# ndoll1998/lightgrad

Hardware: AMD Instinct MI355X
Metric: mnist_mlp_train_steps_per_sec_batch1024_per_gpu (higher is better)
Workload: dtype f32; 1 GPU; mnist_mlp_784x512x10_bias_batch1024_mse_adabelief_lr1e-3 (fwd+bwd+allreduce+optimizer); batch_per_gpu=1024, global_batch=1024, parallelism=dp1, optimizer_kernel=fused, input_requires_grad=True, dispatch=hipGraph replay (python tape captured once; 13 consecutive steps per graph), steps_per_graph=13, device=AMD Instinct (gfx950), compute_units=256, clock_mhz=2400

## Files before the change

include/lghip.h:

```cpp
#ifndef LGHIP_H
#define LGHIP_H

#include <stddef.h>
#include <stdint.h>

#ifdef __cplusplus
extern "C" {
#endif

#define LG_MAX_DIMS 8

#define LG_OK            0
#define LG_EINVAL       -1
#define LG_EHIP         -2
#define LG_ENOMEM       -3
#define LG_ENOTINIT     -4
#define LG_ECOMM        -5
#define LG_EINDEX       -6

const char* lg_last_error(void);

int lg_device_count(int* count);
int lg_init(int device);
int lg_device(int* device);
// ... 221 lines not shown
                              const float* mask, int64_t sbm);
int lg_attention_long_bwd_f32(const float* q, int64_t ldq, int64_t sbq, const float* k, int64_t ldk, int64_t sbk,
                              const float* v, int64_t ldv, int64_t sbv, const float* g, int64_t ldg, int64_t sbg,
                              const float* p, float* dq, int64_t lddq, int64_t sbdq, float* dk, int64_t lddk, int64_t sbdk,
                              float* dv, int64_t lddv, int64_t sbdv, int64_t batch, int64_t heads, int64_t S, int64_t D,
                              float scale);

int lg_attention_dropout_supported(int64_t S, int64_t D);
int lg_attention_dropout_fwd_f32(const float* q, int64_t ldq, int64_t sbq, const float* k, int64_t ldk, int64_t sbk,
                                 const float* v, int64_t ldv, int64_t sbv, float* o, int64_t ldo, int64_t sbo, float* p,
                                 int64_t batch, int64_t heads, int64_t S, int64_t D, float scale,
                                 const float* mask, int64_t sbm, double prob, uint64_t* base_out);
int lg_attention_dropout_bwd_f32(const float* q, int64_t ldq, int64_t sbq, const float* k, int64_t ldk, int64_t sbk,
                                 const float* v, int64_t ldv, int64_t sbv, const float* g, int64_t ldg, int64_t sbg,
                                 const float* p, float* dq, int64_t lddq, int64_t sbdq, float* dk, int64_t lddk, int64_t sbdk,
                                 float* dv, int64_t lddv, int64_t sbdv, int64_t batch, int64_t heads, int64_t S, int64_t D,
                                 float scale, double prob, const uint64_t* base);

int lg_gemm_pair_begin(void);
int lg_gemm_pair_end(void);
int lg_gemm_pair_mse_loss(const float* row_loss, int64_t rows, int64_t n, float* loss);
int lg_gemm_pair_hold(void);
int lg_gemm_pair_resume(void);

int lg_gemm_group_begin(void);
int lg_gemm_group_colsum_f32(const float* in, int64_t ld, int64_t rows, int64_t cols, float* out, int accumulate);
int lg_gemm_group_flush(void);
int lg_gemm_group_end(void);

int lg_head_fwd_f32(const float* x, int64_t ldx, int relu, const float* w, const float* bias, const float* target,
                    float* y, float* err, float* row_loss, int64_t rows, int64_t hidden, int64_t outs);
int lg_head_fwd_grad_f32(const float* x, int64_t ldx, int relu, const float* w, const float* bias, const float* target,
                         float* y, float* err, float* row_loss, float* dx, float* gpre, int64_t rows, int64_t hidden, int64_t outs);
int lg_gemm_bias_head_fwd_f32(const float* x, int64_t ldx, const float* w1, int64_t ldw1, const float* b1, float* pre,
                              int64_t rows, int64_t hidden, int64_t d_in, int relu,
                              const float* w2, const float* b2, const float* target, float* y, float* err, float* row_loss,
                              float* dx, float* gpre, int64_t outs, int chain, int* launches);
int lg_mse_finalize_f32(const float* row_loss, int64_t rows, int64_t n, float* loss);
int lg_head_bwd_f32(const float* x, int64_t ldx, int relu, const float* g, const float* w,
                    float* dx, float* gpre, float* dw, int dw_accumulate, float* db, int db_accumulate,
                    int64_t rows, int64_t hidden, int64_t outs, const float* row_loss, float* loss);

int lg_softmax_f32(const float* x, float* y, int64_t rows, int64_t cols);
int lg_softmax_bwd_f32(const float* y, const float* g, float* dx, int64_t rows, int64_t cols);
int lg_softmax_scaled_f32(const float* x, float* y, int64_t rows, int64_t cols, float scale);
int lg_softmax_scaled_bwd_f32(const float* y, const float* g, float* dx, int64_t rows, int64_t cols, float scale);
// ... 59 lines not shown
```

lightgrad_amd/autograd/hip/lib.py:

```python
import ctypes
import os
from ctypes import c_int, c_int64, c_uint32, c_uint64, c_size_t, c_float, c_double, c_void_p, c_char_p, POINTER

_PKG_DIR = os.path.dirname(os.path.dirname(os.path.dirname(os.path.abspath(__file__))))
LIB_PATH = os.environ.get("LIGHTGRAD_HIP_LIB") or os.path.join(_PKG_DIR, "liblghip.so")
COMM_LIB_PATH = os.path.join(_PKG_DIR, "liblghip_comm.so")

ACT_GELU, ACT_GELU_BWD = 1, 2
EW_COPY, EW_NEG, EW_EXP, EW_LOG, EW_RELU, EW_SIGMOID, EW_TANH, EW_SIN, EW_COS, EW_SQRT, EW_GELU = range(11)
(EW_ADD, EW_SUB, EW_MUL, EW_DIV, EW_POW, EW_RELU_BWD, EW_SIGMOID_BWD, EW_TANH_BWD, EW_LOG_BWD,
 EW_SIN_BWD, EW_COS_BWD, EW_EQ, EW_GE, EW_BIAS_RELU, EW_GELU_BWD) = range(32, 47)
EW_MAX_BWD, EW_FMA = 64, 65
EW_MUL_BWD, EW_DIV_BWD, EW_POW_BWD = 96, 97, 98
RED_SUM, RED_MAX, RED_MIN = 0, 1, 2
DT_I16, DT_I32, DT_I64, DT_F64, DT_F32 = 1, 2, 3, 4, 5


class DeviceInfo(ctypes.Structure):
    _fields_ = [("name", ctypes.c_char * 128), ("arch", ctypes.c_char * 32),
                ("compute_units", ctypes.c_int32), ("clock_mhz", ctypes.c_int32),
                ("wavefront_size", ctypes.c_int32), ("lds_bytes_per_cu", ctypes.c_int32),
                ("hbm_bytes", ctypes.c_uint64), ("l2_bytes", ctypes.c_int32), ("reserved", ctypes.c_int32)]


# ... 30 lines not shown
    "lg_fill_strided": (c_int, [c_int, c_int, _I64P, c_void_p, _I64P, c_uint64]),
    "lg_ew": (c_int, [c_int, c_int, _I64P, c_void_p, _I64P, c_void_p, _I64P,
                      c_void_p, _I64P, c_void_p, _I64P, c_void_p, _I64P, c_void_p, _I64P, c_float]),
    "lg_ew_last_plan": (c_int, [POINTER(ctypes.c_int32)]),
    "lg_reduce": (c_int, [c_int, c_int, _I64P, c_void_p, _I64P, c_uint32, c_void_p]),
    "lg_ew_typed": (c_int, [c_int, c_int, c_int, _I64P, c_void_p, _I64P, c_void_p, _I64P, c_void_p, _I64P, c_double, c_int64]),
    "lg_reduce_typed": (c_int, [c_int, c_int, c_int, _I64P, c_void_p, _I64P, c_uint32, c_void_p]),
    "lg_cast": (c_int, [c_int, c_int, c_int, _I64P, c_void_p, _I64P, c_void_p, _I64P]),
    "lg_reduce_acc": (c_int, [c_int, c_int, _I64P, c_void_p, _I64P, c_uint32, c_void_p, c_int]),
    "lg_reduce_last_plan": (c_int, [POINTER(ctypes.c_int32)]),
    "lg_argreduce_f32": (c_int, [c_int, c_int, _I64P, c_void_p, _I64P, c_int, c_void_p]),
    "lg_argreduce_last_plan": (c_int, [POINTER(ctypes.c_int32)]),
    "lg_top1_count_f32": (c_int, [c_void_p, c_int64, c_int64, c_void_p, c_int, c_int, c_int64, c_int, c_void_p]),
    "lg_gemm_f32": (c_int, [c_int, c_int, c_int64, c_int64, c_int64, c_void_p, c_int64, c_int64,
                            c_void_p, c_int64, c_int64, c_void_p, c_int64, c_int64, c_int64, c_int]),
    "lg_gemm_bf16_f32": (c_int, [c_int, c_int, c_int64, c_int64, c_int64, c_void_p, c_int64, c_void_p, c_int64, c_void_p, c_int64,
                                 c_void_p, c_int]),
    "lg_bf16_round_f32": (c_int, [c_void_p, c_void_p, c_int64]),
    "lg_gemm_pair_begin": (c_int, []),
    "lg_gemm_pair_end": (c_int, []),
    "lg_gemm_pair_mse_loss": (c_int, [c_void_p, c_int64, c_int64, c_void_p]),
    "lg_gemm_pair_hold": (c_int, []),
    "lg_gemm_pair_resume": (c_int, []),
    "lg_gemm_group_begin": (c_int, []),
    "lg_gemm_group_colsum_f32": (c_int, [c_void_p, c_int64, c_int64, c_int64, c_void_p, c_int]),
    "lg_gemm_group_flush": (c_int, []),
    "lg_gemm_group_end": (c_int, []),
    "lg_adam_step_f32": (c_int, [c_void_p, c_void_p, c_void_p, c_void_p, c_int64, c_double, c_double, c_double,
                                 c_double, c_double, c_double, c_double, c_int]),
    "lg_adam_step_dev_f32": (c_int, [c_void_p, c_void_p, c_void_p, c_void_p, c_int64, c_double, c_double, c_double,
                                     c_double, c_void_p, c_int64, c_int64, c_double, c_int]),
    "lg_counter_add_i64": (c_int, [c_void_p, c_int64]),
    "lg_adam_multi_dev_f32": (c_int, [c_void_p, c_void_p, c_void_p, c_void_p, c_int, _I64P, c_double, c_double, c_double,
                                      c_double, c_void_p, c_int64, c_double, c_int]),
    "lg_grad_norm_clip_f32": (c_int, [c_void_p, c_int64, c_double, c_double, c_void_p, c_void_p, c_void_p]),
    "lg_adamw_multi_dev_f32": (c_int, [c_void_p, c_void_p, c_void_p, c_void_p, c_int, _I64P, c_double, c_double, c_double,
                                       c_double, c_void_p, c_int64, c_double, c_int, c_double, c_char_p, c_void_p, c_int, c_int64, c_int64]),
    "lg_adam_plan_create": (c_int, [POINTER(c_void_p), c_void_p, c_void_p, c_void_p, c_void_p, c_int64, c_void_p, c_void_p, c_int64, c_int64,
                                    c_double, c_double, c_double, c_double, c_double, c_int]),
    "lg_adam_plan_destroy": (c_int, [c_void_p]),
    "lg_adam_epilogue_arm": (c_int, [c_void_p, c_int64, c_void_p]),
    "lg_adam_epilogue_finish": (c_int, [POINTER(c_int), POINTER(c_int)]),
    "lg_adam_epilogue_disarm": (c_int, []),
    "lg_gemm_bias_f32": (c_int, [c_int, c_int, c_int64, c_int64, c_int64, c_void_p, c_int64, c_int64,
                                 c_void_p, c_int64, c_int64, c_void_p, c_int64, c_int64, c_int64, c_void_p]),
    "lg_gemm_addend_f32": (c_int, [c_int, c_int, c_int64, c_int64, c_int64, c_void_p, c_int64, c_void_p, c_int64, c_void_p, c_int64,
# ... 180 lines not shown
```

lightgrad_amd/csrc/gemm.hip:

```cpp
#include "common.h"
#include "gelu_common.h"
#include "adam_common.h"
#include "tail_jobs.h"
#include "mse_finalize.h"
#include "head_fwd_body.h"
#include <cstdlib>
#include <cstring>
#include <type_traits>

namespace lg {

typedef float f32x16 __attribute__((ext_vector_type(16)));
typedef unsigned int u32x4 __attribute__((ext_vector_type(4)));
typedef float f32x4 __attribute__((ext_vector_type(4)));

#ifndef LG_SMALL_PD
#define LG_SMALL_PD 2
#endif
constexpr int kSmallTilePrefetch = LG_SMALL_PD;
#ifndef LG_WAVE_PRIVATE_PD
#define LG_WAVE_PRIVATE_PD 1
#endif
constexpr int kWavePrivatePrefetch = LG_WAVE_PRIVATE_PD;

// ... 3 lines not shown
};
static FastDiv make_fastdiv(int64_t d) {
    if (d < 1) d = 1;
    uint32_t l = 0;
    while ((int64_t(1) << l) < d) ++l;
    FastDiv f;
    f.m = uint32_t((uint64_t(1) << (31 + l)) / uint64_t(d) + 1);
    f.s = 31 + l;
    return f;
}

struct GemmArgs {
    const float* A;
    const float* B;
    float*       C;
    int64_t M, N, K;
    int64_t lda, ldb, ldc;
    int64_t sA, sB, sC;
    int64_t sA2, sB2, sC2;
    int     batch_inner;
    int     tiles_m, tiles_n;
    int     nwg;
    int     accumulate;
    const float* bias;
    const float* addend;
    int64_t      ldadd;
    int     group_m;
    int     k_slices;
    int64_t k_per_slice;
    float*  W;
    int*    tickets;
    float*  rowsum;
    int     rowsum_accumulate;
    FastDiv div_per_batch, div_slices, div_gspan, div_group, div_last_group, div_batch_inner;
    int     k_tail;
    short   relu_a, relu_b;
    int     act;
    float*  aux;
    int     multi;
    int64_t boff[3], coff[3], biasoff[3];
    int     seg_k, seg_steps;
    int64_t seg_jump[2];
    const AdamPlan* adam_c;
    const AdamPlan* adam_r;
#ifdef LG_GEMM_TIMELINE
    unsigned long long* tl;
// ... 84 lines not shown
            while (__hip_atomic_load(flag, __ATOMIC_RELAXED, __HIP_MEMORY_SCOPE_AGENT) == 0) {
                __builtin_amdgcn_s_sleep(2);
                if (wall_clock64() - t0 > 200000000ull) {
                    __hip_atomic_fetch_or(c.status, LG_STATUS_HANDOFF_TIMEOUT, __ATOMIC_RELAXED, __HIP_MEMORY_SCOPE_SYSTEM);
                    ok = 0;
                    break;
                }
            }
            seen = ok;
        }
        __syncthreads();
        __builtin_amdgcn_fence(__ATOMIC_ACQUIRE, "wavefront");
        const int64_t row = row0 + wave;
        if (row < a.rows) head_fwd_row<OMAX, true>(a, lds, row, lane);
        if (tid == 0 && seen) {
            if (__hip_atomic_fetch_add(done, 1, __ATOMIC_RELAXED, __HIP_MEMORY_SCOPE_AGENT) == readers - 1) {
                __hip_atomic_store(done, 0, __ATOMIC_RELAXED, __HIP_MEMORY_SCOPE_AGENT);
                __hip_atomic_store(flag, 0, __ATOMIC_RELAXED, __HIP_MEMORY_SCOPE_AGENT);
            }
        }
    }
}

template <int PD, bool SECOND_BKC = false>
__global__ void __launch_bounds__(256) sgemm_pair_wgrad_xgrad(GemmArgs first, GemmArgs second) {
    constexpr int L1 = gemm_lds_floats<64, 64, 32, false, false, 1>(), L2 = gemm_lds_floats<64, 64, 32, true, SECOND_BKC, 1>();
    __shared__ __attribute__((aligned(16))) float lds[L1 > L2 ? L1 : L2];
    constexpr int BM = 64, BN = 64, BK = 32, WM = 2, WN = 2, KG = 1, XT = 0;
    constexpr bool VA = true, VB = true;
#define LG_TILE_OWNS_LDS 0
    if (int(blockIdx.x) < first.nwg) {
        constexpr bool AKC = false, BKC = false;
        const GemmArgs& g = first;
#define LG_TILE_BID int(blockIdx.x)
#include "gemm_tile_body.inc"
#undef LG_TILE_BID
    } else {
        constexpr bool AKC = true, BKC = SECOND_BKC;
        const GemmArgs& g = second;
#define LG_TILE_BID (int(blockIdx.x) - first.nwg)
#include "gemm_tile_body.inc"
#undef LG_TILE_BID
    }
#undef LG_TILE_OWNS_LDS
}

int lg_mse_finalize_job(const float* row_loss, int64_t rows, float inv_n, float* loss);
struct PairFirsts { GemmArgs w[2]; };
struct LossJob {
    const float* row_loss;
    float*       loss;
    int64_t      rows;
    float        inv_n;
};
template <int PD>
__global__ void __launch_bounds__(256) sgemm_triple_wgrad2_xgrad(PairFirsts firsts, GemmArgs second, LossJob job) {
    constexpr int L1 = gemm_lds_floats<64, 64, 32, false, false, 1>(), L2 = gemm_lds_floats<64, 64, 32, true, false, 1>();
    __shared__ __attribute__((aligned(16))) float lds[L1 > L2 ? L1 : L2];
    constexpr int BM = 64, BN = 64, BK = 32, WM = 2, WN = 2, KG = 1, XT = 0;
    constexpr bool VA = true, VB = true;
#define LG_TILE_OWNS_LDS 0
    const int n0w = firsts.w[0].nwg, n1w = firsts.w[1].nwg;
    if (int(blockIdx.x) < n0w + n1w) {
        constexpr bool AKC = false, BKC = false;
        const int which = int(blockIdx.x) >= n0w ? 1 : 0;
        const GemmArgs g = firsts.w[which];
#define LG_TILE_BID (int(blockIdx.x) - (which ? n0w : 0))
#include "gemm_tile_body.inc"
#undef LG_TILE_BID
    } else if (int(blockIdx.x) < n0w + n1w + second.nwg) {
        constexpr bool AKC = true, BKC = false;
        const GemmArgs& g = second;
#define LG_TILE_BID (int(blockIdx.x) - n0w - n1w)
#include "gemm_tile_body.inc"
#undef LG_TILE_BID
    } else {
        finalize_loss(job.row_loss, job.rows, job.inv_n, job.loss, lds);
    }
#undef LG_TILE_OWNS_LDS
}

constexpr int kGroupMax = 14;
struct GroupProduct {
    const float* A;
    const float* B;
    float*       C;
    float*       W;
    int*         tickets;
    float*       rowsum;
    int64_t      M, N, K, lda, ldb, ldc, k_per_slice;
    int          tiles_m, tiles_n, nwg, accumulate, group_m, k_slices, rowsum_accumulate, k_tail;
    FastDiv      div_per_batch, div_slices, div_gspan, div_group, div_last_group, div_batch_inner;
// ... 43 lines not shown
        int64_t r = q;
        for (; r + 28 < grp.cs_rows; r += 32) {
#pragma unroll
            for (int e = 0; e < 8; ++e) acc[e] += in[(r + 4 * e) * grp.cs_ld];
        }
        for (; r < grp.cs_rows; r += 4) acc[0] += in[r * grp.cs_ld];
        lds[threadIdx.x] = ((acc[0] + acc[1]) + (acc[2] + acc[3])) + ((acc[4] + acc[5]) + (acc[6] + acc[7]));
        __syncthreads();
        if (q == 0 && live) {
            const float v = (lds[cl] + lds[64 + cl]) + (lds[128 + cl] + lds[192 + cl]);
            grp.cs_out[col] = grp.cs_accumulate ? grp.cs_out[col] + v : v;
        }
        return;
    }
    const int bid = int(blockIdx.x) - grp.cs_wgs;
    if (bid >= grp.first[grp.count]) {
        tail_group_body(grp.tail, bid - grp.first[grp.count]);
        return;
    }
    int which = 0;
    while (which + 1 < grp.count && bid >= grp.first[which + 1]) ++which;
    const GemmArgs g = unpack_product(grp.p[which]);
#define LG_TILE_OWNS_LDS 0
#define LG_TILE_BID (bid - grp.first[which])
#include "gemm_tile_body.inc"
#undef LG_TILE_BID
#undef LG_TILE_OWNS_LDS
}

template <int BM, int BN, int BK, int WM, int WN, bool AKC, bool BKC, int KG>
static void launch_layout(const GemmArgs& g, bool va, bool vb) {
    dim3 grid(g.nwg), block(WM * WN * KG * 64);
    hipStream_t s = rt().stream;
    constexpr int PD = (BM * BN <= 64 * 64) ? kSmallTilePrefetch : 2;
    static_assert(BM * BN < 256 * 256 || PD <= 2, "a third K-tile in flight does not fit the 256x256 tile's 128 registers: ring registers would spill while their loads are in flight");
    if constexpr (kWavePrivateTile<BM, BN, WM, WN, KG> && AKC && BKC) {
        static const char* kloop_env = getenv("LG_GEMM_KLOOP");
        if (va && vb && !(kloop_env && strcmp(kloop_env, "coop") == 0)) {
            constexpr int WPD = kWavePrivatePrefetch;
            if (g.multi) hipLaunchKernelGGL((sgemm_mfma<BM, BN, BK, WM, WN, true, true, true, true, WPD, KG, 1, true>), grid, block, 0, s, g);
            else         hipLaunchKernelGGL((sgemm_mfma<BM, BN, BK, WM, WN, true, true, true, true, WPD, KG, 0, true>), grid, block, 0, s, g);
            return;
        }
    }
    if constexpr (kHasExtras<BM, BN>) {
        if constexpr (AKC && BKC)  { if (g.multi) { hipLaunchKernelGGL((sgemm_mfma<BM, BN, BK, WM, WN, AKC, BKC, true, true, PD, KG, 1>), grid, block, 0, s, g); return; } }
        if constexpr (AKC && !BKC) { if (g.seg_k) { hipLaunchKernelGGL((sgemm_mfma<BM, BN, BK, WM, WN, AKC, BKC, true, true, PD, KG, 2>), grid, block, 0, s, g); return; } }
    }
    if constexpr (!kHasExtras<BM, BN>) {
        hipLaunchKernelGGL((sgemm_mfma<BM, BN, BK, WM, WN, AKC, BKC, true, true, PD, KG>), grid, block, 0, s, g);
        return;
    }
    if (va && vb)  hipLaunchKernelGGL((sgemm_mfma<BM, BN, BK, WM, WN, AKC, BKC, true, true, PD, KG>), grid, block, 0, s, g);
    else if (va)   hipLaunchKernelGGL((sgemm_mfma<BM, BN, BK, WM, WN, AKC, BKC, true, false, 1, KG>), grid, block, 0, s, g);
    else if (vb)   hipLaunchKernelGGL((sgemm_mfma<BM, BN, BK, WM, WN, AKC, BKC, false, true, 1, KG>), grid, block, 0, s, g);
    else           hipLaunchKernelGGL((sgemm_mfma<BM, BN, BK, WM, WN, AKC, BKC, false, false, 1, KG>), grid, block, 0, s, g);
}

#ifdef LG_GEMM_TIMELINE
static void lg_debug_timeline_state(unsigned long long* buf, int nwg, int slices, int tiles);
#endif
struct PairState {
    int      active = 0;
    int      count = 0;
    bool     second_bkc = false;
    GemmArgs args[3];
    bool     is_s[3] = {false, false, false};
    int64_t  batch[3] = {1, 1, 1};
    int64_t  tiles = 0;
    LossJob  job{};
};
static PairState& pair_state() { static PairState p; return p; }

static void pair_launch_single(const GemmArgs& g, bool is_s) {
    dim3 grid(g.nwg), block(256);
    constexpr int PD = kSmallTilePrefetch;
    if (!is_s) hipLaunchKernelGGL((sgemm_mfma<64, 64, 32, 2, 2, false, false, true, true, PD, 1>), grid, block, 0, rt().stream, g);
    else if (pair_state().second_bkc) hipLaunchKernelGGL((sgemm_mfma<64, 64, 32, 2, 2, true, true, true, true, PD, 1>), grid, block, 0, rt().stream, g);
    else           hipLaunchKernelGGL((sgemm_mfma<64, 64, 32, 2, 2, true, false, true, true, PD, 1>), grid, block, 0, rt().stream, g);
}

static int pair_retune(GemmArgs& g, int64_t others_nwg) {
    const int64_t tiles = int64_t(g.tiles_m) * g.tiles_n;
    static const char* pair_slices_env = getenv("LG_GEMM_PAIR_SLICES");
    if (pair_slices_env || g.nwg != tiles * g.k_slices || g.seg_k || tiles >= 256 || g.K < 128) return LG_OK;
    constexpr int BK = 32, BM = 64, BN = 64;
    const double cus = rt().compute_units > 0 ? rt().compute_units : 256;
    const int64_t k_tiles = (g.K + BK - 1) / BK;
    int64_t best_sl = g.k_slices;
    double best = 1e30;
    for (int64_t sl = 1; sl <= 64 && (sl == 1 || sl * 2 <= k_tiles); ++sl) {
        const double per_cu = double(tiles * sl + others_nwg) / cus;
        const double c = per_cu > 1.0 ? double(int64_t(per_cu + 0.999)) : 1.0;
        const double cost = double((k_tiles + sl - 1) / sl) * (c <= 1.0 ? 0.68 : 0.43 * c + 0.17) + (sl > 1 ? 1.8 + 0.85 * double(sl) : 0.0);
        if (cost < best) { best = cost; best_sl = sl; }
    }
    int64_t k_per_slice = ((g.K + best_sl - 1) / best_sl + BK - 1) / BK * BK;
    best_sl = (g.K + k_per_slice - 1) / k_per_slice;
    if (best_sl == g.k_slices) return LG_OK;
    if (g.W) { const int rc = lg_free(g.W); g.W = nullptr; if (rc != LG_OK) return rc; }
    g.k_per_slice = k_per_slice;
    g.k_slices = int(best_sl);
    g.nwg = int(tiles * best_sl);
    g.div_slices = make_fastdiv(best_sl);
    if (best_sl > 1) {
        const int rc = lg_malloc(reinterpret_cast<void**>(&g.W), size_t(tiles * best_sl) * BM * BN * sizeof(float));
        if (rc != LG_OK) return rc;
    }
    return LG_OK;
}

static int pair_flush(bool keep_collecting) {
    PairState& P = pair_state();
    int rc = LG_OK;
    bool job_done = false;
    if (P.count == 3) {
        rc = pair_retune(P.args[1], int64_t(P.args[0].nwg) + P.args[2].nwg);
        if (rc != LG_OK) { P.count = 0; return rc; }
        PairFirsts firsts;
        firsts.w[0] = P.args[0];
        firsts.w[1] = P.args[1];
        const int spare = P.job.loss ? 1 : 0;
        hipLaunchKernelGGL((sgemm_triple_wgrad2_xgrad<kSmallTilePrefetch>), dim3(P.args[0].nwg + P.args[1].nwg + P.args[2].nwg + spare), dim3(256), 0,
                           rt().stream, firsts, P.args[2], P.job);
        job_done = true;
    } else if (P.count == 2 && P.is_s[1]) {
        rc = pair_retune(P.args[0], P.args[1].nwg);
        if (rc != LG_OK) { P.count = 0; return rc; }
#ifdef LG_GEMM_TIMELINE
        if (P.args[0].tl) {
            (void)hipMemsetAsync(P.args[0].tl, 0, size_t(P.args[0].nwg + P.args[1].nwg) * 64, rt().stream);
            lg_debug_timeline_state(P.args[0].tl, P.args[0].nwg + P.args[1].nwg, P.args[0].k_slices * 100 + P.args[1].k_slices, P.args[0].nwg);
        }
#endif
        if (P.second_bkc)
            hipLaunchKernelGGL((sgemm_pair_wgrad_xgrad<kSmallTilePrefetch, true>), dim3(P.args[0].nwg + P.args[1].nwg), dim3(256), 0, rt().stream,
                               P.args[0], P.args[1]);
        else
            hipLaunchKernelGGL((sgemm_pair_wgrad_xgrad<kSmallTilePrefetch, false>), dim3(P.args[0].nwg + P.args[1].nwg), dim3(256), 0, rt().stream,
                               P.args[0], P.args[1]);
    } else {
        for (int i = 0; i < P.count; ++i) pair_launch_single(P.args[i], P.is_s[i]);
    }
    for (int i = 0; i < P.count; ++i)
        if (P.args[i].W) { const int r = lg_free(P.args[i].W); if (r != LG_OK) rc = r; }
    P.count = 0;
    P.tiles = 0;
    if (job_done) P.job = LossJob{};
    if (!keep_collecting && P.active) P.active = 2;
    return rc;
}

struct WriteSpan { uintptr_t lo, hi; };
static WriteSpan product_c_span(const GemmArgs& g, int64_t batch) {
    const int64_t outer = batch / g.batch_inner;
    int64_t lo = 0, hi = (g.M - 1) * g.ldc + g.N;
    const int64_t reach[2] = {(outer - 1) * g.sC, int64_t(g.batch_inner - 1) * g.sC2};
    for (int64_t r : reach) { if (r < 0) lo += r; else hi += r; }
    const uintptr_t base = reinterpret_cast<uintptr_t>(g.C);
    return WriteSpan{base + uintptr_t(lo * 4), base + uintptr_t(hi * 4)};
}
static bool spans_meet(WriteSpan a, WriteSpan b) { return a.lo < b.hi && b.lo < a.hi; }
static bool products_write_alike(const GemmArgs& a, int64_t batch_a, const GemmArgs& b, int64_t batch_b) {
// ... 94 lines not shown
    } else if (clash || G.count == kGroupMax || G.tiles + tiles > rt().n_gemm_tickets / 2) {
        rc = group_flush();
        if (rc != LG_OK) return false;
    }
    g.tickets = rt().gemm_tickets + G.tiles;
    G.tiles += tiles;
    G.queued[G.count] = g;
    G.count += 1;
    return true;
}

bool gemm_group_is_open() { return group_state().active == 1; }

int gemm_group_flush_pending() {
    if (pair_state().count) { const int prc = pair_flush(true); if (prc != LG_OK) return prc; }
    const int rc = group_flush();
    const int rc2 = ln_group_flush_pending();
    return rc != LG_OK ? rc : rc2;
}

#ifdef LG_GEMM_TIMELINE
static unsigned long long* g_tl_buf = nullptr;
static int g_tl_nwg = 0, g_tl_slices = 0, g_tl_tiles = 0;
static void lg_debug_timeline_state(unsigned long long* buf, int nwg, int slices, int tiles) {
    g_tl_buf = buf; g_tl_nwg = nwg; g_tl_slices = slices; g_tl_tiles = tiles;
}
#endif

template <int BM, int BN, int BK, int WM, int WN, int KG = 1>
static int launch_config(const GemmArgs& base, bool akc, bool bkc, bool va, bool vb, int64_t batch) {
    GemmArgs g = base;
    g.tiles_m = int((g.M + BM - 1) / BM);
    g.tiles_n = int((g.N + (g.rowsum ? 1 : 0) + BN - 1) / BN);
    const int64_t tiles = int64_t(g.tiles_m) * g.tiles_n * batch;
    int64_t slices = 1;
    if (kCanSplitK<BM, BN, KG> && tiles < 256 && g.K >= 4 * BK) {
        const double cus = rt().compute_units > 0 ? rt().compute_units : 256;
        const double t_iter = BM * BN >= 128 * 128 ? 2.4 : (BM * BN >= 64 * 64 ? 0.65 : 0.45);
        const int64_t k_tiles = (g.K + BK - 1) / BK;
        double best = 1e30;
        for (int64_t sl = 1; sl <= 64 && sl * 2 <= k_tiles; ++sl) {
            const double per_cu = double(tiles * sl) / cus;
            const double kt = double((k_tiles + sl - 1) / sl);
            double cost;
            if (BM * BN == 64 * 64) {
                const double c = per_cu > 1.0 ? double(int64_t(per_cu + 0.999)) : 1.0;
                cost = kt * (c <= 1.0 ? 0.68 : 0.43 * c + 0.17) + (sl > 1 ? 1.8 + 0.85 * double(sl) : 0.0);
            } else {
                cost = kt * t_iter * (per_cu > 1.0 ? per_cu : 1.0) + (sl > 1 ? 2.0 + 0.6 * double(sl) : 0.0);
            }
            if (cost < best) { best = cost; slices = sl; }
        }
    }
    static const char* slices_env = getenv("LG_GEMM_SLICES");
    if (kCanSplitK<BM, BN, KG> && slices_env && atoi(slices_env) >= 1) slices = atoi(slices_env);
    static const char* pair_slices_env = getenv("LG_GEMM_PAIR_SLICES");
    if (kCanSplitK<BM, BN, KG> && pair_slices_env && pair_state().active == 1) {
        int sv[3] = {0, 0, 0};
        const int got = sscanf(pair_slices_env, "%d,%d,%d", &sv[0], &sv[1], &sv[2]);
        if (got >= 2) { const int c = pair_state().count; const int v = c < got ? sv[c] : sv[got - 1]; if (v >= 1) slices = v; }
    }
    if (g.seg_k) { slices = 1; g.seg_steps = g.seg_k / (BK * KG); }
    g.k_per_slice = ((g.K + slices - 1) / slices + BK - 1) / BK * BK;
    slices = (g.K + g.k_per_slice - 1) / g.k_per_slice;
    g.k_slices = int(slices);
    g.nwg = int(tiles * slices);
    g.div_per_batch = make_fastdiv(int64_t(g.tiles_m) * g.tiles_n);
    g.div_slices = make_fastdiv(slices);
    g.div_gspan = make_fastdiv(int64_t(g.group_m) * g.tiles_n);
    g.div_group = make_fastdiv(g.group_m);
    g.div_last_group = make_fastdiv(g.tiles_m % g.group_m ? g.tiles_m % g.group_m : g.group_m);
    g.div_batch_inner = make_fastdiv(g.batch_inner);
    g.W = nullptr;
    g.tickets = rt().gemm_tickets;
#ifdef LG_GEMM_TIMELINE
    {
        static unsigned long long* tl_buf = nullptr;
        if (!tl_buf) (void)hipMalloc(reinterpret_cast<void**>(&tl_buf), size_t(1) << 22);
        g.tl = (tl_buf && size_t(g.nwg) * 64 <= (size_t(1) << 22)) ? tl_buf : nullptr;
        if (g.tl) (void)hipMemsetAsync(g.tl, 0, size_t(g.nwg) * 64, rt().stream);
        lg_debug_timeline_state(tl_buf, g.nwg, g.k_slices, int(tiles));
    }
#endif
    if (slices > 1 && tiles > rt().n_gemm_tickets) {
        slices = 1;
        g.k_per_slice = (g.K + BK - 1) / BK * BK;
        g.k_slices = 1;
        g.nwg = int(tiles);
        g.div_slices = make_fastdiv(1);
    }
    if (slices > 1) {
        int rc = lg_malloc(reinterpret_cast<void**>(&g.W), size_t(tiles * slices) * BM * BN * sizeof(float));
        if (rc != LG_OK) return rc;
    }
    if constexpr (BM == 64 && BN == 64 && WM == 2 && WN == 2 && KG == 1) {
        if (pair_try_defer(g, akc, bkc, va, vb, batch)) return LG_OK;
        int grc = LG_OK;
// ... 250 lines not shown
    return gemm_impl(transA, transB, M, N, K, A, lda, strideA_outer, B, ldb, strideB_outer, C, ldc, strideC_outer,
                     batch_outer * batch_inner, accumulate, nullptr, nullptr, 0, batch_inner, strideA_inner, strideB_inner, strideC_inner);
}

extern "C" int lg_gemm_fused_f32(int transA, int transB, int64_t M, int64_t N, int64_t K,
                                 const float* A, int64_t lda, const float* B, int64_t ldb, float* C, int64_t ldc,
                                 int accumulate, const float* bias, float* rowsum, int rowsum_accumulate,
                                 int relu_a, int relu_b) {
    LG_ARG(!(bias && rowsum), "lg_gemm_fused_f32: bias and rowsum exclude each other");
    LG_ARG(!(bias && accumulate), "lg_gemm_fused_f32: bias and accumulate exclude each other");
    return gemm_impl(transA, transB, M, N, K, A, lda, 0, B, ldb, 0, C, ldc, 0, 1, accumulate, bias, rowsum, rowsum_accumulate,
                     1, 0, 0, 0, relu_a, relu_b);
}

#ifdef LG_GEMM_TIMELINE
extern "C" int lg_debug_gemm_timeline(unsigned long long* host, int max_wgs, int* nwg, int* slices, int* tiles) {
    LG_REQUIRE_INIT();
    LG_HIP(hipStreamSynchronize(rt().stream));
    const int n = lg::g_tl_nwg < max_wgs ? lg::g_tl_nwg : max_wgs;
    if (lg::g_tl_buf && n > 0) LG_HIP(hipMemcpy(host, lg::g_tl_buf, size_t(n) * 64, hipMemcpyDeviceToHost));
    *nwg = n; *slices = lg::g_tl_slices; *tiles = lg::g_tl_tiles;
    return LG_OK;
}
#endif

extern "C" int lg_gemm_pair_begin(void) {
    LG_REQUIRE_INIT();
    PairState& P = lg::pair_state();
    LG_ARG(P.active == 0, "lg_gemm_pair_begin: a pair bracket is already open");
    P.active = 1;
    P.count = 0;
    return LG_OK;
}

extern "C" int lg_gemm_pair_end(void) {
    LG_REQUIRE_INIT();
    PairState& P = lg::pair_state();
    LG_ARG(P.active != 0, "lg_gemm_pair_end: no pair bracket is open");
    int rc = lg::pair_flush(true);
    P.active = 0;
    if (P.job.loss) {
        const int r = lg::lg_mse_finalize_job(P.job.row_loss, P.job.rows, P.job.inv_n, P.job.loss);
        P.job = lg::LossJob{};
        if (r != LG_OK) rc = r;
    }
    if (rc != LG_OK) return rc;
    LG_CHECK_LAUNCH();
    return LG_OK;
}

extern "C" int lg_gemm_pair_hold(void) {
    LG_REQUIRE_INIT();
    PairState& P = lg::pair_state();
    LG_ARG(P.active == 1 || P.active == 2, "lg_gemm_pair_hold: no pair bracket is open");
    if (P.active == 1) P.active = 3;
    return LG_OK;
}

extern "C" int lg_gemm_pair_resume(void) {
    LG_REQUIRE_INIT();
    PairState& P = lg::pair_state();
    LG_ARG(P.active != 0, "lg_gemm_pair_resume: no pair bracket is open");
    if (P.active == 3) P.active = 1;
    return LG_OK;
}

extern "C" int lg_gemm_pair_mse_loss(const float* row_loss, int64_t rows, int64_t n, float* loss) {
    LG_REQUIRE_INIT();
    PairState& P = lg::pair_state();
    LG_ARG(P.active != 0, "lg_gemm_pair_mse_loss: no pair bracket is open");
// ... 100 lines not shown
```

lightgrad_amd/csrc/gemm_tile_body.inc:

```
#ifndef LG_TILE_SIGNAL
#define LG_TILE_SIGNAL 0
#endif
#ifndef LG_TILE_WAVE_PRIVATE
#define LG_TILE_WAVE_PRIVATE false
#endif
    constexpr bool WPK = LG_TILE_WAVE_PRIVATE;
    static_assert(!WPK || (KG > 1 && WM * WN == 1 && BM == 32 && BN == 32 && AKC && BKC && VA && VB && XT != 2 && !LG_TILE_SIGNAL), "wave-private K loop: one wave per K-group, NT form");
    constexpr int NT = WM * WN * KG * 64;
    constexpr int NTS = WPK ? 64 : NT;
    constexpr int BKS = WPK ? BK : BK * KG;
    constexpr int TM = BM / WM / 32, TN = BN / WN / 32;
    static_assert(TM >= 1 && TN >= 1 && BK % 16 == 0 && (KG == 1 || KG == 2 || KG == 4), "tile config");
    constexpr bool AG = kGatherStaging<BM, BN, AKC>, BG = kGatherStaging<BM, BN, BKC>;
    static_assert((!AG || VA) && (!BG || VB), "gather staging replaces the float4 form");
    constexpr bool ALK = AKC || AG, BLK = BKC || BG;
    constexpr int A_PITCH = ALK ? BKS + 4 : BM;
    constexpr int B_PITCH = BLK ? BKS + 4 : BN;
    constexpr int A_TILE = ALK ? BM * A_PITCH : BKS * A_PITCH;
    constexpr int B_TILE = BLK ? BN * B_PITCH : BKS * B_PITCH;
    constexpr int A_ELEMS = BM * BKS / NTS, B_ELEMS = BN * BKS / NTS;
    static_assert(A_ELEMS % 4 == 0 && B_ELEMS % 4 == 0, "staging must divide into float4");

    static_assert(WPK || 2 * (A_TILE + B_TILE) == gemm_lds_floats<BM, BN, BK, AKC, BKC, KG>(), "LDS size");
    static_assert(!(AG || BG) || TM * TN > 1, "gather staging: the multi-accumulator loop only");
#if LG_TILE_OWNS_LDS
    __shared__ __attribute__((aligned(16))) float lds[gemm_lds_floats<BM, BN, BK, AKC, BKC, KG>()];
#endif
// ... 422 lines not shown
        for (int kt0 = 0; kt0 < nkt; kt0 += PD) {
    #pragma unroll
            for (int u = 0; u < PD; ++u) {
                const int kt = kt0 + u;
                if (kt < nkt) {
                    const int cur = kt & 1;
                    if (PD == 1 && kt + 1 < nkt) load_tile(0);
                    compute_tile(cur, 0, BK / 2);
                    if (kt + 1 < nkt) {
                        int younger = nkt - (kt + 2);
                        if (younger > PD - 2) younger = PD - 2;
                        wait_tile((u + 1) % PD, PD == 1 ? 0 : (younger < 0 ? 0 : younger));
                        store_tile(cur ^ 1, (u + 1) % PD);
                    }
                    if (PD > 1 && kt + PD < nkt) load_tile(u);
                    compute_tile(cur, BK / 2, BK);
                    __syncthreads();
                }
            }
        }
    }

    LG_TL(2);
    if constexpr (KG > 1) {
        constexpr int GROUP_FLOATS = WM * WN * TM * TN * 16 * 64;
        static_assert(WPK || (KG - 1) * GROUP_FLOATS <= 2 * (A_TILE + B_TILE), "the K-group exchange must fit the staging buffers");
        static_assert(!WPK || KG * BUF + (KG - 1) * GROUP_FLOATS <= gemm_lds_floats<BM, BN, BK, AKC, BKC, KG>(), "staging regions + exchange");
        float* x = lds + (WPK ? KG * BUF : 0) + (wl * TM * TN * 16) * 64 + lane;
        if (kg >= 1) {
#pragma unroll
            for (int i = 0; i < TM; ++i)
#pragma unroll
                for (int j = 0; j < TN; ++j)
#pragma unroll
                    for (int e = 0; e < 16; ++e) x[(kg - 1) * GROUP_FLOATS + ((i * TN + j) * 16 + e) * 64] = acc[i][j][e];
        }
        __syncthreads();
        if (kg >= 1) return;
#pragma unroll
        for (int gq = 0; gq < KG - 1; ++gq)
#pragma unroll
            for (int i = 0; i < TM; ++i)
#pragma unroll
                for (int j = 0; j < TN; ++j)
#pragma unroll
                    for (int e = 0; e < 16; ++e) acc[i][j][e] += x[gq * GROUP_FLOATS + ((i * TN + j) * 16 + e) * 64];
    }
    [[maybe_unused]] AdamScalars adam_cs_c, adam_cs_r;
    [[maybe_unused]] int64_t adam_done_c = 0, adam_done_r = 0;
    if constexpr (kCanAdam<BM, BN, KG>) {
        if (g.adam_c) adam_cs_c = adam_plan_scalars(g.adam_c, adam_done_c);
        if (g.adam_r) adam_cs_r = adam_plan_scalars(g.adam_r, adam_done_r);
    }
    if constexpr (kCanSplitK<BM, BN, KG>) if (g.k_slices > 1) {
        constexpr int SC1 = 16;
        constexpr int TILE_BYTES = BM * BN * 4;
        char* slab0 = reinterpret_cast<char*>(g.W) + (int64_t(batch) * g.k_slices * per_batch + t) * int64_t(TILE_BYTES);
        const int64_t slice_stride = int64_t(per_batch) * TILE_BYTES;
        {
            const auto mine = __builtin_amdgcn_make_buffer_rsrc(slab0 + slice * slice_stride, 0, TILE_BYTES, 0x00020000);
#pragma unroll
            for (int i = 0; i < TM; ++i)
#pragma unroll
                for (int j = 0; j < TN; ++j)
#pragma unroll
                    for (int q = 0; q < 4; ++q) {
                        u32x4 v;
#pragma unroll
                        for (int e = 0; e < 4; ++e) v[e] = __float_as_uint(acc[i][j][4 * q + e]);
                        __builtin_amdgcn_raw_buffer_store_b128(v, mine, (((i * TN + j) * 4 + q) * NT + tid) * 16, 0, SC1);
                    }
        }
        asm volatile("s_waitcnt vmcnt(0)" ::: "memory");
        __syncthreads();
        LG_TL(3);
        int* arrived_last = reinterpret_cast<int*>(lds);
        if (tid == 0) {
            int* ticket = g.tickets + batch * per_batch + t;
            const int order = __hip_atomic_fetch_add(ticket, 1, __ATOMIC_RELAXED, __HIP_MEMORY_SCOPE_AGENT);
            const int last = order == g.k_slices - 1;
            if (last) __hip_atomic_store(ticket, 0, __ATOMIC_RELAXED, __HIP_MEMORY_SCOPE_AGENT);
            *arrived_last = last;
        }
        __syncthreads();
        LG_TL(4);
        if (!*arrived_last) return;
        __builtin_amdgcn_fence(__ATOMIC_ACQUIRE, "wavefront");
        constexpr int CH = TM * TN >= 4 ? 1 : (TM * TN == 2 ? 2 : 4);
        for (int s0 = 0; s0 < g.k_slices; s0 += CH) {
            u32x4 v[CH][TM * TN * 4];
#pragma unroll
            for (int c = 0; c < CH; ++c) {
                const int sl = s0 + c < g.k_slices ? s0 + c : s0;
                const auto src = __builtin_amdgcn_make_buffer_rsrc(slab0 + sl * slice_stride, 0, TILE_BYTES, 0x00020000);
#pragma unroll
                for (int f = 0; f < TM * TN * 4; ++f) v[c][f] = __builtin_amdgcn_raw_buffer_load_b128(src, (f * NT + tid) * 16, 0, SC1);
            }
#pragma unroll
            for (int c = 0; c < CH; ++c) {
                const bool live = s0 + c < g.k_slices, first = s0 + c == 0;
#pragma unroll
                for (int i = 0; i < TM; ++i)
#pragma unroll
                    for (int j = 0; j < TN; ++j)
#pragma unroll
                        for (int e = 0; e < 16; ++e) {
                            const float w = __uint_as_float(v[c][(i * TN + j) * 4 + e / 4][e % 4]);
                            acc[i][j][e] = first ? w : (live ? acc[i][j][e] + w : acc[i][j][e]);
                        }
            }
        }
// ... 102 lines not shown
                }
            }
        }
    }
    if constexpr (kCanAdam<BM, BN, KG>) {
        if (tid == 0 && tm == 0) {
            if (g.adam_c && tn == 0 && g.adam_c->step_out)
                __hip_atomic_store(g.adam_c->step_out, adam_done_c + 1, __ATOMIC_RELAXED, __HIP_MEMORY_SCOPE_AGENT);
            if (g.adam_r && has_virtual && g.adam_r->step_out)
                __hip_atomic_store(g.adam_r->step_out, adam_done_r + 1, __ATOMIC_RELAXED, __HIP_MEMORY_SCOPE_AGENT);
        }
    }
    LG_TL(6);
#if LG_TILE_SIGNAL
    asm volatile("s_waitcnt vmcnt(0)" ::: "memory");
    if (lane == 0) {
        int* const ticket = signal_tickets + tm * signal_stride;
        if (__hip_atomic_fetch_add(ticket, 1, __ATOMIC_RELAXED, __HIP_MEMORY_SCOPE_AGENT) == signal_per_row - 1) {
            __hip_atomic_store(ticket, 0, __ATOMIC_RELAXED, __HIP_MEMORY_SCOPE_AGENT);
            __hip_atomic_store(ticket + 16, 1, __ATOMIC_RELAXED, __HIP_MEMORY_SCOPE_AGENT);
        }
    }
#endif
```

Baseline: 21280 steps/s.

## Fold own split-K partial from LDS and add wave-priority backward scheduling

In the split-K reduction, the last-arriving workgroup keeps its own partial tile in LDS and folds it in instead of rereading it from the global slab. This removes one global slice reload per reduced tile, and the fold is on by default. The change also adds optional s_setprio wave priorities for the weight-gradient GEMMs in the pair and triple backward kernels, plus APIs to force split-K slice counts. Priority defaults to 0, so that part is inactive unless configured; the fold changes the order of floating-point summation and adds LDS traffic.

```diff
diff --git a/include/lghip.h b/include/lghip.h
--- a/include/lghip.h
+++ b/include/lghip.h
@@ -267,6 +267,10 @@
 int lg_gemm_pair_mse_loss(const float* row_loss, int64_t rows, int64_t n, float* loss);
 int lg_gemm_pair_hold(void);
 int lg_gemm_pair_resume(void);
+int lg_gemm_backward_schedule(int wgrad_priority, int wgrad_priority_drop, int pair_priority, int fold_own);
+int lg_gemm_backward_schedule_get(int* settings);
+int lg_gemm_pair_slices(int first, int second, int third);
+int lg_gemm_pair_last_slices(int* products, int* k_slices);
 
 int lg_gemm_group_begin(void);
 int lg_gemm_group_colsum_f32(const float* in, int64_t ld, int64_t rows, int64_t cols, float* out, int accumulate);
diff --git a/lightgrad_amd/autograd/hip/lib.py b/lightgrad_amd/autograd/hip/lib.py
--- a/lightgrad_amd/autograd/hip/lib.py
+++ b/lightgrad_amd/autograd/hip/lib.py
@@ -76,6 +76,10 @@
     "lg_gemm_pair_mse_loss": (c_int, [c_void_p, c_int64, c_int64, c_void_p]),
     "lg_gemm_pair_hold": (c_int, []),
     "lg_gemm_pair_resume": (c_int, []),
+    "lg_gemm_backward_schedule": (c_int, [c_int, c_int, c_int, c_int]),
+    "lg_gemm_backward_schedule_get": (c_int, [c_void_p]),
+    "lg_gemm_pair_slices": (c_int, [c_int, c_int, c_int]),
+    "lg_gemm_pair_last_slices": (c_int, [c_void_p, c_void_p]),
     "lg_gemm_group_begin": (c_int, []),
     "lg_gemm_group_colsum_f32": (c_int, [c_void_p, c_int64, c_int64, c_int64, c_void_p, c_int]),
     "lg_gemm_group_flush": (c_int, []),
diff --git a/lightgrad_amd/csrc/gemm.hip b/lightgrad_amd/csrc/gemm.hip
--- a/lightgrad_amd/csrc/gemm.hip
+++ b/lightgrad_amd/csrc/gemm.hip
@@ -49,6 +49,7 @@
     int     tiles_m, tiles_n;
     int     nwg;
     int     accumulate;
+    int     fold_own;
     const float* bias;
     const float* addend;
     int64_t      ldadd;
@@ -179,8 +180,31 @@
     }
 }
 
+constexpr int kWgradPrio = 0;
+struct BackwardSchedule { int triple_prio, pair_prio, fold_own; };
+static int parse_prio(const char* e, int dflt) {
+    if (!e || e[0] < '0' || e[0] > '3') return dflt;
+    return (e[0] - '0') | ((e[1] == 'd' && e[0] != '0') ? 4 : 0);
+}
+static BackwardSchedule& backward_schedule() {
+    static BackwardSchedule s = [] {
+        const char* f = getenv("LG_GEMM_FOLD_OWN");
+        return BackwardSchedule{parse_prio(getenv("LG_GEMM_WGRAD_PRIO"), kWgradPrio), parse_prio(getenv("LG_GEMM_PAIR_PRIO"), 0),
+                                (f && f[0] == '0') ? 0 : 1};
+    }();
+    return s;
+}
+static int (&forced_pair_slices())[3] { static int v[3] = {0, 0, 0}; return v; }
+static int (&last_shared_launch())[4] { static int v[4] = {0, 0, 0, 0}; return v; }
+__device__ __forceinline__ void raise_wave_priority(int sched) {
+    const int level = sched & 3;
+    if (level == 1) __builtin_amdgcn_s_setprio(1);
+    else if (level == 2) __builtin_amdgcn_s_setprio(2);
+    else if (level == 3) __builtin_amdgcn_s_setprio(3);
+}
+
 template <int PD, bool SECOND_BKC = false>
-__global__ void __launch_bounds__(256) sgemm_pair_wgrad_xgrad(GemmArgs first, GemmArgs second) {
+__global__ void __launch_bounds__(256) sgemm_pair_wgrad_xgrad(GemmArgs first, GemmArgs second, int sched) {
     constexpr int L1 = gemm_lds_floats<64, 64, 32, false, false, 1>(), L2 = gemm_lds_floats<64, 64, 32, true, SECOND_BKC, 1>();
     __shared__ __attribute__((aligned(16))) float lds[L1 > L2 ? L1 : L2];
     constexpr int BM = 64, BN = 64, BK = 32, WM = 2, WN = 2, KG = 1, XT = 0;
@@ -189,9 +213,13 @@
     if (int(blockIdx.x) < first.nwg) {
         constexpr bool AKC = false, BKC = false;
         const GemmArgs& g = first;
+        raise_wave_priority(sched);
+#undef LG_TILE_KLOOP_DONE
+#define LG_TILE_KLOOP_DONE() do { if (sched & 4) __builtin_amdgcn_s_setprio(0); } while (0)
 #define LG_TILE_BID int(blockIdx.x)
 #include "gemm_tile_body.inc"
 #undef LG_TILE_BID
+#undef LG_TILE_KLOOP_DONE
     } else {
         constexpr bool AKC = true, BKC = SECOND_BKC;
         const GemmArgs& g = second;
@@ -203,7 +231,7 @@
 }
 
 int lg_mse_finalize_job(const float* row_loss, int64_t rows, float inv_n, float* loss);
-struct PairFirsts { GemmArgs w[2]; };
+struct PairFirsts { GemmArgs w[2]; int sched; };
 struct LossJob {
     const float* row_loss;
     float*       loss;
@@ -222,9 +250,14 @@
         constexpr bool AKC = false, BKC = false;
         const int which = int(blockIdx.x) >= n0w ? 1 : 0;
         const GemmArgs g = firsts.w[which];
+        const int sched = firsts.sched;
+        raise_wave_priority(sched);
+#undef LG_TILE_KLOOP_DONE
+#define LG_TILE_KLOOP_DONE() do { if (sched & 4) __builtin_amdgcn_s_setprio(0); } while (0)
 #define LG_TILE_BID (int(blockIdx.x) - (which ? n0w : 0))
 #include "gemm_tile_body.inc"
 #undef LG_TILE_BID
+#undef LG_TILE_KLOOP_DONE
     } else if (int(blockIdx.x) < n0w + n1w + second.nwg) {
         constexpr bool AKC = true, BKC = false;
         const GemmArgs& g = second;
@@ -314,9 +347,11 @@
     while (which + 1 < grp.count && bid >= grp.first[which + 1]) ++which;
     const GemmArgs g = unpack_product(grp.p[which]);
 #define LG_TILE_OWNS_LDS 0
+#define LG_TILE_FOLD_OWN 0
 #define LG_TILE_BID (bid - grp.first[which])
 #include "gemm_tile_body.inc"
 #undef LG_TILE_BID
+#undef LG_TILE_FOLD_OWN
 #undef LG_TILE_OWNS_LDS
 }
 
@@ -351,6 +386,7 @@
 
 #ifdef LG_GEMM_TIMELINE
 static void lg_debug_timeline_state(unsigned long long* buf, int nwg, int slices, int tiles);
+static void lg_debug_timeline_roles(int n0, int n1, int n2, int s0, int s1, int s2);
 #endif
 struct PairState {
     int      active = 0;
@@ -375,7 +411,7 @@
 static int pair_retune(GemmArgs& g, int64_t others_nwg) {
     const int64_t tiles = int64_t(g.tiles_m) * g.tiles_n;
     static const char* pair_slices_env = getenv("LG_GEMM_PAIR_SLICES");
-    if (pair_slices_env || g.nwg != tiles * g.k_slices || g.seg_k || tiles >= 256 || g.K < 128) return LG_OK;
+    if (pair_slices_env || forced_pair_slices()[0] || g.nwg != tiles * g.k_slices || g.seg_k || tiles >= 256 || g.K < 128) return LG_OK;
     constexpr int BK = 32, BM = 64, BN = 64;
     const double cus = rt().compute_units > 0 ? rt().compute_units : 256;
     const int64_t k_tiles = (g.K + BK - 1) / BK;
@@ -412,13 +448,26 @@
         PairFirsts firsts;
         firsts.w[0] = P.args[0];
         firsts.w[1] = P.args[1];
+        firsts.sched = backward_schedule().triple_prio;
         const int spare = P.job.loss ? 1 : 0;
+        { int (&ls)[4] = last_shared_launch(); ls[0] = 3; for (int i = 0; i < 3; ++i) ls[1 + i] = P.args[i].k_slices; }
+#ifdef LG_GEMM_TIMELINE
+        const int n0 = P.args[0].nwg, n1 = P.args[1].nwg, n2 = P.args[2].nwg;
+        if (P.args[0].tl && P.args[1].tl && P.args[2].tl && size_t(n0 + n1 + n2 + spare) * 64 <= (size_t(1) << 22)) {
+            (void)hipMemsetAsync(P.args[0].tl, 0, size_t(n0 + n1 + n2 + spare) * 64, rt().stream);
+            lg_debug_timeline_state(P.args[0].tl, n0 + n1 + n2, P.args[1].k_slices * 100 + P.args[2].k_slices, n0 + n1);
+            lg_debug_timeline_roles(n0, n1, n2, P.args[0].k_slices, P.args[1].k_slices, P.args[2].k_slices);
+        } else {
+            firsts.w[0].tl = firsts.w[1].tl = P.args[2].tl = nullptr;
+        }
+#endif
         hipLaunchKernelGGL((sgemm_triple_wgrad2_xgrad<kSmallTilePrefetch>), dim3(P.args[0].nwg + P.args[1].nwg + P.args[2].nwg + spare), dim3(256), 0,
                            rt().stream, firsts, P.args[2], P.job);
         job_done = true;
     } else if (P.count == 2 && P.is_s[1]) {
         rc = pair_retune(P.args[0], P.args[1].nwg);
         if (rc != LG_OK) { P.count = 0; return rc; }
+        { int (&ls)[4] = last_shared_launch(); ls[0] = 2; ls[1] = P.args[0].k_slices; ls[2] = P.args[1].k_slices; ls[3] = 0; }
 #ifdef LG_GEMM_TIMELINE
         if (P.args[0].tl) {
             (void)hipMemsetAsync(P.args[0].tl, 0, size_t(P.args[0].nwg + P.args[1].nwg) * 64, rt().stream);
@@ -427,10 +476,10 @@
 #endif
         if (P.second_bkc)
             hipLaunchKernelGGL((sgemm_pair_wgrad_xgrad<kSmallTilePrefetch, true>), dim3(P.args[0].nwg + P.args[1].nwg), dim3(256), 0, rt().stream,
-                               P.args[0], P.args[1]);
+                               P.args[0], P.args[1], backward_schedule().pair_prio);
         else
             hipLaunchKernelGGL((sgemm_pair_wgrad_xgrad<kSmallTilePrefetch, false>), dim3(P.args[0].nwg + P.args[1].nwg), dim3(256), 0, rt().stream,
-                               P.args[0], P.args[1]);
+                               P.args[0], P.args[1], backward_schedule().pair_prio);
     } else {
         for (int i = 0; i < P.count; ++i) pair_launch_single(P.args[i], P.is_s[i]);
     }
@@ -571,8 +620,14 @@
 #ifdef LG_GEMM_TIMELINE
 static unsigned long long* g_tl_buf = nullptr;
 static int g_tl_nwg = 0, g_tl_slices = 0, g_tl_tiles = 0;
+static int g_tl_roles[6] = {0, 0, 0, 0, 0, 0};
 static void lg_debug_timeline_state(unsigned long long* buf, int nwg, int slices, int tiles) {
     g_tl_buf = buf; g_tl_nwg = nwg; g_tl_slices = slices; g_tl_tiles = tiles;
+    for (int i = 0; i < 6; ++i) g_tl_roles[i] = 0;
+}
+static void lg_debug_timeline_roles(int n0, int n1, int n2, int s0, int s1, int s2) {
+    const int v[6] = {n0, n1, n2, s0, s1, s2};
+    for (int i = 0; i < 6; ++i) g_tl_roles[i] = v[i];
 }
 #endif
 
@@ -609,6 +664,10 @@
         const int got = sscanf(pair_slices_env, "%d,%d,%d", &sv[0], &sv[1], &sv[2]);
         if (got >= 2) { const int c = pair_state().count; const int v = c < got ? sv[c] : sv[got - 1]; if (v >= 1) slices = v; }
     }
+    if (kCanSplitK<BM, BN, KG> && forced_pair_slices()[0] && pair_state().active == 1) {
+        const int v = forced_pair_slices()[pair_state().count < 3 ? pair_state().count : 2];
+        if (v >= 1) slices = v;
+    }
     if (g.seg_k) { slices = 1; g.seg_steps = g.seg_k / (BK * KG); }
     g.k_per_slice = ((g.K + slices - 1) / slices + BK - 1) / BK * BK;
     slices = (g.K + g.k_per_slice - 1) / g.k_per_slice;
@@ -622,6 +681,7 @@
     g.div_batch_inner = make_fastdiv(g.batch_inner);
     g.W = nullptr;
     g.tickets = rt().gemm_tickets;
+    g.fold_own = backward_schedule().fold_own;
 #ifdef LG_GEMM_TIMELINE
     {
         static unsigned long long* tl_buf = nullptr;
@@ -918,6 +978,10 @@
     *nwg = n; *slices = lg::g_tl_slices; *tiles = lg::g_tl_tiles;
     return LG_OK;
 }
+extern "C" int lg_debug_gemm_timeline_roles(int* roles) {
+    for (int i = 0; i < 6; ++i) roles[i] = lg::g_tl_roles[i];
+    return LG_OK;
+}
 #endif
 
 extern "C" int lg_gemm_pair_begin(void) {
@@ -942,6 +1006,39 @@
     }
     if (rc != LG_OK) return rc;
     LG_CHECK_LAUNCH();
+    return LG_OK;
+}
+
+extern "C" int lg_gemm_backward_schedule(int wgrad_priority, int wgrad_priority_drop, int pair_priority, int fold_own) {
+    LG_ARG(wgrad_priority <= 3 && pair_priority <= 3, "lg_gemm_backward_schedule: priorities are 0..3 (negative: unchanged)");
+    lg::BackwardSchedule& s = lg::backward_schedule();
+    if (wgrad_priority >= 0) s.triple_prio = wgrad_priority | ((wgrad_priority_drop > 0 && wgrad_priority > 0) ? 4 : 0);
+    if (pair_priority >= 0) s.pair_prio = pair_priority;
+    if (fold_own >= 0) s.fold_own = fold_own ? 1 : 0;
+    return LG_OK;
+}
+
+extern "C" int lg_gemm_backward_schedule_get(int* settings) {
+    LG_ARG(settings, "lg_gemm_backward_schedule_get: NULL pointer");
+    const lg::BackwardSchedule& s = lg::backward_schedule();
+    settings[0] = s.triple_prio & 3; settings[1] = (s.triple_prio & 4) ? 1 : 0; settings[2] = s.pair_prio & 3; settings[3] = s.fold_own;
+    return LG_OK;
+}
+
+extern "C" int lg_gemm_pair_slices(int first, int second, int third) {
+    LG_ARG(first >= 0 && second >= 0 && third >= 0 && first <= 64 && second <= 64 && third <= 64, "lg_gemm_pair_slices: counts are 0 (the model's choice) .. 64");
+    LG_ARG(first > 0 || (second == 0 && third == 0), "lg_gemm_pair_slices: all three counts or none");
+    int (&v)[3] = lg::forced_pair_slices();
+    v[0] = first; v[1] = second ? second : first; v[2] = third ? third : v[1];
+    if (!first) v[1] = v[2] = 0;
+    return LG_OK;
+}
+
+extern "C" int lg_gemm_pair_last_slices(int* products, int* k_slices) {
+    LG_ARG(products && k_slices, "lg_gemm_pair_last_slices: NULL pointer");
+    const int (&ls)[4] = lg::last_shared_launch();
+    *products = ls[0];
+    for (int i = 0; i < 3; ++i) k_slices[i] = ls[1 + i];
     return LG_OK;
 }
 
diff --git a/lightgrad_amd/csrc/gemm_tile_body.inc b/lightgrad_amd/csrc/gemm_tile_body.inc
--- a/lightgrad_amd/csrc/gemm_tile_body.inc
+++ b/lightgrad_amd/csrc/gemm_tile_body.inc
@@ -3,6 +3,13 @@
 #endif
 #ifndef LG_TILE_WAVE_PRIVATE
 #define LG_TILE_WAVE_PRIVATE false
+#endif
+#ifndef LG_TILE_KLOOP_DONE
+#define LG_TILE_KLOOP_DONE() do { } while (0)
+#endif
+#ifndef LG_TILE_FOLD_OWN
+#define LG_TILE_FOLD_OWN 1
+#define LG_TILE_FOLD_OWN_DEFAULTED
 #endif
     constexpr bool WPK = LG_TILE_WAVE_PRIVATE;
     static_assert(!WPK || (KG > 1 && WM * WN == 1 && BM == 32 && BN == 32 && AKC && BKC && VA && VB && XT != 2 && !LG_TILE_SIGNAL), "wave-private K loop: one wave per K-group, NT form");
@@ -471,6 +478,7 @@
     }
 
     LG_TL(2);
+    LG_TILE_KLOOP_DONE();
     if constexpr (KG > 1) {
         constexpr int GROUP_FLOATS = WM * WN * TM * TN * 16 * 64;
         static_assert(WPK || (KG - 1) * GROUP_FLOATS <= 2 * (A_TILE + B_TILE), "the K-group exchange must fit the staging buffers");
@@ -506,6 +514,18 @@
         constexpr int TILE_BYTES = BM * BN * 4;
         char* slab0 = reinterpret_cast<char*>(g.W) + (int64_t(batch) * g.k_slices * per_batch + t) * int64_t(TILE_BYTES);
         const int64_t slice_stride = int64_t(per_batch) * TILE_BYTES;
+        constexpr bool FOLD_OWN = LG_TILE_FOLD_OWN && TM * TN == 1 && BM == 64 && BN == 64 && VA && VB && (AKC || !BKC);
+        bool fold_own = false;
+        [[maybe_unused]] float* const own_lds = lds + 64;
+        if constexpr (FOLD_OWN) {
+            static_assert(64 + NT * 16 <= 2 * (A_TILE + B_TILE), "the own copy must fit the staging buffers");
+            fold_own = g.fold_own != 0;
+            if (fold_own) {
+#pragma unroll
+                for (int q = 0; q < 4; ++q)
+                    *reinterpret_cast<f32x4*>(own_lds + (q * NT + tid) * 4) = f32x4{acc[0][0][4 * q], acc[0][0][4 * q + 1], acc[0][0][4 * q + 2], acc[0][0][4 * q + 3]};
+            }
+        }
         {
             const auto mine = __builtin_amdgcn_make_buffer_rsrc(slab0 + slice * slice_stride, 0, TILE_BYTES, 0x00020000);
 #pragma unroll
@@ -536,6 +556,60 @@
         if (!*arrived_last) return;
         __builtin_amdgcn_fence(__ATOMIC_ACQUIRE, "wavefront");
         constexpr int CH = TM * TN >= 4 ? 1 : (TM * TN == 2 ? 2 : 4);
+        if (fold_own) {
+            if constexpr (FOLD_OWN) {
+                const int others = g.k_slices - 1;
+                auto for_own = [&](auto&& f) {
+                    int at = tid * 4;
+#pragma unroll
+                    for (int q = 0; q < 4; ++q) {
+                        asm volatile("" : "+v"(at));
+                        const f32x4 r = f(q, *reinterpret_cast<const f32x4*>(own_lds + q * NT * 4 + at));
+                        float r0 = r[0], r1 = r[1], r2 = r[2], r3 = r[3];
+                        asm volatile("" : "+v"(at), "+v"(r0), "+v"(r1), "+v"(r2), "+v"(r3));
+                        acc[0][0][4 * q] = r0; acc[0][0][4 * q + 1] = r1; acc[0][0][4 * q + 2] = r2; acc[0][0][4 * q + 3] = r3;
+                    }
+                };
+                auto batch = [&](auto n, int j0) {
+                    constexpr int N = decltype(n)::value;
+                    u32x4 v[N][4];
+#pragma unroll
+                    for (int c = 0; c < N; ++c) {
+                        const int j = j0 + c < others ? j0 + c : j0;
+                        const int sl = j < slice ? j : j + 1;
+                        const auto src = __builtin_amdgcn_make_buffer_rsrc(slab0 + sl * slice_stride, 0, TILE_BYTES, 0x00020000);
+#pragma unroll
+                        for (int f = 0; f < 4; ++f) v[c][f] = __builtin_amdgcn_raw_buffer_load_b128(src, tid * 16, f * NT * 16, SC1);
+                    }
+#pragma unroll
+                    for (int c = 0; c < N; ++c) {
+                        const int j = j0 + c;
+                        if (j < others) {
+                            if (j == 0 && slice == 0) {
+                                for_own([&](int q, f32x4 o) {
+                                    return f32x4{o[0] + __uint_as_float(v[c][q][0]), o[1] + __uint_as_float(v[c][q][1]),
+                                                 o[2] + __uint_as_float(v[c][q][2]), o[3] + __uint_as_float(v[c][q][3])};
+                                });
+                            } else {
+                                const bool first = j == 0;
+#pragma unroll
+                                for (int e = 0; e < 16; ++e) {
+                                    const float w = __uint_as_float(v[c][e / 4][e % 4]);
+                                    acc[0][0][e] = first ? w : acc[0][0][e] + w;
+                                }
+                            }
+                            if (j + 1 == slice) {
+                                for_own([&](int q, f32x4 o) {
+                                    return f32x4{acc[0][0][4 * q] + o[0], acc[0][0][4 * q + 1] + o[1], acc[0][0][4 * q + 2] + o[2], acc[0][0][4 * q + 3] + o[3]};
+                                });
+                            }
+                        }
+                    }
+                };
+                batch(std::integral_constant<int, CH>(), 0);
+                for (int j0 = CH; j0 < others; j0 += CH - 1) batch(std::integral_constant<int, CH - 1>(), j0);
+            }
+        } else
         for (int s0 = 0; s0 < g.k_slices; s0 += CH) {
             u32x4 v[CH][TM * TN * 4];
 #pragma unroll
@@ -684,3 +758,7 @@
         }
     }
 #endif
+#ifdef LG_TILE_FOLD_OWN_DEFAULTED
+#undef LG_TILE_FOLD_OWN
+#undef LG_TILE_FOLD_OWN_DEFAULTED
+#endif
```

Result: no change. 21280 steps/s (-0.0%).
